# ivanalberico/End-To-End-Self-Supervised-SLAM

Measured on AMD Instinct MI355X. Metric: online refinement steps/sec @640x480, seq_len=60, higher is better.
Workload: dtype f32

## Files before the change

### end-to-end-self-supervised-slam_amd/csrc/conv.hip

```cpp
#include <cassert>
#include <type_traits>

#include "e2e_common.h"

typedef float f4v __attribute__((ext_vector_type(4)));
typedef float f16v __attribute__((ext_vector_type(16)));

#define CBK 16

enum { ACT_NONE = 0, ACT_RELU = 1, ACT_ELU = 2, ACT_DISP = 3 };

struct ConvArgs {
    const float* src0;
    const float* src1;
    const float* w;
    const float* scale;
    const float* shift;
    const float* res;
    float* out;
    int B, Hs, Ws;
    int Cin, C1, up;
    int Hd, Wd;
    int Ncols, ldw;
    int KH, KW, stride, pad, pad_mode;
// ... 1760 lines not shown
#pragma unroll
        for (int i = 0; i < 5; ++i) {
            const int f = tid + TAP_NT * i;
            if (f < 800) *(f4v*)&xs[f * 4] = rx[i];
        }
    };
    if (c_begin < c_end) load_chunk(c_begin);
    const float* ap = dzs + kh_ * 32 + l32;
    const float* bp = xs + (kh_ + wave * 10) * 32 + l32;
    for (int c = c_begin; c < c_end; ++c) {
        __syncthreads();
        store_chunk();
        __syncthreads();
        if (c + 1 < c_end) load_chunk(c + 1);
        constexpr int QB = 4, NQ = 32 / QB;
        float av[2][QB], bv[2][QB][3];
        auto read_q = [&](int set, int qt) {
#pragma unroll
            for (int j = 0; j < QB; ++j) {
                const int ks = QB * qt + j, q0 = (ks >> 2) * 10 + 2 * (ks & 3);
                av[set][j] = ap[2 * ks * 32];
#pragma unroll
                for (int t = 0; t < 3; ++t) bv[set][j][t] = bp[(q0 + t) * 32];
            }
        };
        auto pin_q = [&](int set) {
#pragma unroll
            for (int j = 0; j < QB; ++j) {
                asm volatile("" : "+v"(av[set][j]));
#pragma unroll
                for (int t = 0; t < 3; ++t) asm volatile("" : "+v"(bv[set][j][t]));
            }
        };
        read_q(0, 0);
#pragma unroll
        for (int qt = 0; qt < NQ; ++qt) {
            if (qt + 1 < NQ) read_q((qt + 1) & 1, qt + 1);
            __builtin_amdgcn_sched_barrier(0);
            pin_q(qt & 1);
            __builtin_amdgcn_sched_barrier(0);
#pragma unroll
            for (int j = 0; j < QB; ++j) {
#pragma unroll
                for (int t = 0; t < 3; ++t) acc[t] = __builtin_amdgcn_mfma_f32_32x32x2f32(av[qt & 1][j], bv[qt & 1][j][t], acc[t], 0, 0, 0);
                if (BIAS && want_bias) accb = __builtin_amdgcn_mfma_f32_32x32x2f32(av[qt & 1][j], one, accb, 0, 0, 0);
            }
            __builtin_amdgcn_sched_barrier(0);
        }
    }
    float* slab = a.slabs + (int64_t)blockIdx.z * a.Mpad * a.Npad;
#pragma unroll
    for (int t = 0; t < 3; ++t)
#pragma unroll
        for (int r = 0; r < 16; ++r) {
            const int m = co0 + (r & 3) + 8 * (r >> 2) + 4 * kh_;
            slab[(int64_t)m * a.Npad + (wave * 3 + t) * a.Cin + ci0 + l32] = acc[t][r];
        }
    if (BIAS && want_bias && l32 == 0) {
#pragma unroll
        for (int r = 0; r < 16; ++r) slab[(int64_t)(co0 + (r & 3) + 8 * (r >> 2) + 4 * kh_) * a.Npad + 9 * a.Cin] = accb[r];
    }
}

template <int ZL>
__device__ __forceinline__ void wgrad_reduce_group(const float* __restrict__ slabs, int S, int Mpad, int Npad, int Cout, int Cin, int KH, int KW, int has_bias,
                                                   float* __restrict__ dw, float* __restrict__ dbias, int accumulate, const float* __restrict__ scale,
                                                   int64_t base, int e, int w, f4v (*part)[64]) {
    const int Kconv = KH * KW * Cin, Ng = Kconv + (has_bias ? 1 : 0);
    const int nq = (Ng + 3) / 4;
    const int64_t totalq = (int64_t)Cout * nq;
    const int64_t slab_q = (int64_t)Mpad * Npad / 4;
    const f4v zero = {0.f, 0.f, 0.f, 0.f};
    const int64_t q = base + e;
    const bool on = q < totalq;
    const int m = on ? (int)(q / nq) : 0, n = on ? (int)(q - (int64_t)m * nq) * 4 : 0;
    const f4v* src = (const f4v*)(slabs + (int64_t)m * Npad + n);
    f4v sacc = zero;
    int z = w;
    for (; z + 3 * ZL < S; z += 4 * ZL) {
        f4v v[4];
#pragma unroll
        for (int j = 0; j < 4; ++j) v[j] = on ? src[(int64_t)(z + ZL * j) * slab_q] : zero;
#pragma unroll
        for (int j = 0; j < 4; ++j) sacc += v[j];
    }
    for (; z < S; z += ZL) sacc += on ? src[(int64_t)z * slab_q] : zero;
    part[w][e] = sacc;
    __syncthreads();
    if (w == 0 && on) {
        f4v t = part[0][e];
#pragma unroll
        for (int j = 1; j < ZL; ++j) t += part[j][e];
        const float sc = scale ? scale[m] : 1.f;
#pragma unroll
        for (int k = 0; k < 4; ++k) {
            const int nn = n + k;
            if (nn < Kconv) {
                const int tap = nn / Cin, ci = nn - tap * Cin, kh = tap / KW, kw = tap - kh * KW;
                float* d = dw + (((int64_t)m * Cin + ci) * KH + kh) * KW + kw;
                const float v = scale ? t[k] * sc : t[k];
                *d = accumulate ? *d + v : v;
            } else if (nn == Kconv && dbias) {
                dbias[m] = accumulate ? dbias[m] + t[k] : t[k];
            }
        }
    }
    __syncthreads();
}

template <int ZL>
__global__ __launch_bounds__(64 * ZL) void k_wgrad_reduce(const float* __restrict__ slabs, int S, int Mpad, int Npad, int Cout, int Cin,
                                                         int KH, int KW, int has_bias, float* __restrict__ dw, float* __restrict__ dbias,
                                                         int accumulate, const float* __restrict__ scale) {
    __shared__ f4v part[ZL][64];
    const int64_t totalq = (int64_t)Cout * ((KH * KW * Cin + (has_bias ? 1 : 0) + 3) / 4);
    for (int64_t base = (int64_t)blockIdx.x * 64; base < totalq; base += (int64_t)gridDim.x * 64)
        wgrad_reduce_group<ZL>(slabs, S, Mpad, Npad, Cout, Cin, KH, KW, has_bias, dw, dbias, accumulate, scale, base, threadIdx.x & 63, threadIdx.x >> 6, part);
}

__global__ __launch_bounds__(512) void k_wgrad_reduce_batched(const e2e_wgrad_reduce_desc* __restrict__ d, int n, long long total_items) {
    __shared__ f4v part[8][64];
    const int e = threadIdx.x & 63, w = threadIdx.x >> 6;
    for (long long item = blockIdx.x; item < total_items; item += gridDim.x) {
        int lo = 0, hi = n - 1;
        while (lo < hi) {
            const int mid = (lo + hi + 1) >> 1;
            if (d[mid].first_item <= item) lo = mid; else hi = mid - 1;
        }
        const e2e_wgrad_reduce_desc D = d[lo];
        const long long local = item - D.first_item;
        if (D.zl == 8)
            wgrad_reduce_group<8>(D.slabs, D.S, D.Mpad, D.Npad, D.Cout, D.Cin, D.KH, D.KW, D.has_bias, D.dw, D.dbias, D.accumulate, D.scale, local * 64, e, w, part);
        else
            wgrad_reduce_group<2>(D.slabs, D.S, D.Mpad, D.Npad, D.Cout, D.Cin, D.KH, D.KW, D.has_bias, D.dw, D.dbias, D.accumulate, D.scale,
                                  (local * 4 + (w >> 1)) * 64, e, w & 1, part + 2 * (w >> 1));
    }
}

__global__ __launch_bounds__(256) void k_weight_layouts(const float* __restrict__ w, int Cout, int Cin, int KH, int KW,
                                                        float* __restrict__ wf, int ldf, float* __restrict__ wb, int ldb) {
    const int64_t total = (int64_t)Cout * Cin * KH * KW;
    for (int64_t i = (int64_t)blockIdx.x * 256 + threadIdx.x; i < total; i += (int64_t)gridDim.x * 256) {
        int64_t t = i;
        const int kw = (int)(t % KW); t /= KW;
        const int kh = (int)(t % KH); t /= KH;
        const int ci = (int)(t % Cin); t /= Cin;
        const int co = (int)t;
        const float v = w[i];
        if (wf) wf[((int64_t)(kh * KW + kw) * Cin + ci) * ldf + co] = v;
        if (wb) wb[((int64_t)(kh * KW + kw) * Cout + co) * ldb + ci] = v;
    }
}

__global__ __launch_bounds__(256) void k_weight_layouts_batched(const long long* __restrict__ desc) {
    const long long* d = desc + (int64_t)blockIdx.y * 10;
    const float* __restrict__ w = (const float*)d[0];
    float* __restrict__ wf = (float*)d[1];
    float* __restrict__ wb = (float*)d[2];
    const int Cout = (int)d[3], Cin = (int)d[4], KH = (int)d[5], KW = (int)d[6], ldf = (int)d[7], ldb = (int)d[8];
    const float* __restrict__ bsc = (const float*)d[9];
    const int T = KH * KW;
    constexpr int TMAX = 9, TS = 32;
    __shared__ float tile[TMAX][TS + 1][TS + 1];
    if (T > TMAX) {
        const int64_t total = (int64_t)Cout * Cin * T;
        for (int64_t i = (int64_t)blockIdx.x * 256 + threadIdx.x; i < total; i += (int64_t)gridDim.x * 256) {
            const int tap = (int)(i % T);
            const int64_t r = i / T;
            const int ci = (int)(r % Cin), co = (int)(r / Cin);
            const float v = w[i];
            if (wf) wf[((int64_t)tap * Cin + ci) * ldf + co] = v;
            if (wb) wb[((int64_t)tap * Cout + co) * ldb + ci] = bsc ? v * bsc[co] : v;
        }
        return;
    }
    const int nct = (Cout + TS - 1) / TS, nit = (Cin + TS - 1) / TS;
    for (int t = blockIdx.x; t < nct * nit; t += gridDim.x) {
        const int co0 = (t / nit) * TS, ci0 = (t % nit) * TS;
        const int nci = min(TS, Cin - ci0), nco = min(TS, Cout - co0);
        const int row = nci * T;
        for (int e = threadIdx.x; e < nco * row; e += 256) {
            const int co_l = e / row, rem = e - co_l * row;
            const int ci_l = rem / T, tap = rem - ci_l * T;
            tile[tap][co_l][ci_l] = w[((int64_t)(co0 + co_l) * Cin + ci0) * T + rem];
        }
        __syncthreads();
        if (wf)
            for (int e = threadIdx.x; e < T * nci * nco; e += 256) {
                const int co_l = e % nco, r = e / nco;
                const int ci_l = r % nci, tap = r / nci;
                wf[((int64_t)tap * Cin + ci0 + ci_l) * ldf + co0 + co_l] = tile[tap][co_l][ci_l];
            }
        if (wb)
            for (int e = threadIdx.x; e < T * nco * nci; e += 256) {
                const int ci_l = e % nci, r = e / nci;
                const int co_l = r % nco, tap = r / nco;
                wb[((int64_t)tap * Cout + co0 + co_l) * ldb + ci0 + ci_l] = bsc ? tile[tap][co_l][ci_l] * bsc[co0 + co_l] : tile[tap][co_l][ci_l];
            }
        __syncthreads();
    }
}

__global__ __launch_bounds__(256) void k_act_bwd(const float* __restrict__ dy, const float* __restrict__ y, const float* __restrict__ scale,
                                                 float* __restrict__ dz, int64_t n, int C, int act, int accumulate) {
    for (int64_t i = (int64_t)blockIdx.x * 256 + threadIdx.x; i < n; i += (int64_t)gridDim.x * 256) {
        float g = dy[i];
        const float v = y[i];
        if (act == ACT_RELU) g = v > 0.f ? g : 0.f;
        else if (act == ACT_ELU) g = v > 0.f ? g : g * (v + 1.f);
        else if (act == ACT_DISP) { const float s = (v - 0.01f) * 0.1f; g = g * 10.f * s * (1.f - s); }
        if (scale) g *= scale[i % C];
        dz[i] = accumulate ? dz[i] + g : g;
    }
}

__global__ __launch_bounds__(256) void k_gather_adjoint(const float* __restrict__ dxp, int B, int Hs, int Ws, int Cin, int C1, int up,
                                                        int pp, float* __restrict__ d0, float* __restrict__ d1, int acc0, int acc1,
                                                        const float* __restrict__ x0, int act0, const float* __restrict__ x1, int act1) {
    const int Hp = Hs + 2 * pp, Wp = Ws + 2 * pp, C2 = Cin - C1, Hl = Hs / up, Wl = Ws / up;
    const int64_t n0 = (int64_t)B * Hl * Wl * C1, n1 = (int64_t)B * Hs * Ws * C2;
    for (int64_t i = (int64_t)blockIdx.x * 256 + threadIdx.x; i < n0 + n1; i += (int64_t)gridDim.x * 256) {
        const bool first = i < n0;
        int64_t t = first ? i : i - n0;
        const int Cx = first ? C1 : C2, Hx = first ? Hl : Hs, Wx = first ? Wl : Ws, u = first ? up : 1;
        const int c = (int)(t % Cx); t /= Cx;
        const int x = (int)(t % Wx); t /= Wx;
        const int y = (int)(t % Hx); t /= Hx;
        const int b = (int)t;
        const int cc = first ? c : C1 + c;
        float s = 0.f;
        for (int dy = 0; dy < u; ++dy)
            for (int dx = 0; dx < u; ++dx) {
                const int fy = y * u + dy, fx = x * u + dx;
                int ys[3] = {fy + pp, -1, -1}, xs[3] = {fx + pp, -1, -1};
                if (pp) {
                    if (fy == 1) ys[1] = 0;
                    if (fy == Hs - 2) ys[2] = Hp - 1;
                    if (fx == 1) xs[1] = 0;
                    if (fx == Ws - 2) xs[2] = Wp - 1;
                }
                for (int iy = 0; iy < 3; ++iy)
                    for (int ix = 0; ix < 3; ++ix)
                        if (ys[iy] >= 0 && xs[ix] >= 0) s += dxp[(((int64_t)b * Hp + ys[iy]) * Wp + xs[ix]) * Cin + cc];
            }
        float* d = first ? d0 + i : d1 + (i - n0);
        const int acc = first ? acc0 : acc1;
        if (first ? act0 : act1) s *= act_deriv(first ? x0[i] : x1[i - n0], first ? act0 : act1);
        *d = acc ? *d + s : s;
    }
}

__global__ __launch_bounds__(256) void k_gather_adjoint4(const float* __restrict__ dxp, int B, int Hs, int Ws, int Cin, int C1, int up,
                                                         int pp, float* __restrict__ d0, float* __restrict__ d1, int acc0, int acc1,
                                                         const float* __restrict__ x0, int act0, const float* __restrict__ x1, int act1) {
    const int Hp = Hs + 2 * pp, Wp = Ws + 2 * pp, C2 = Cin - C1, Hl = Hs / up, Wl = Ws / up;
    const unsigned q0 = (unsigned)B * Hl * Wl * (C1 >> 2), q1 = (unsigned)B * Hs * Ws * (C2 >> 2);
    for (unsigned i = blockIdx.x * 256u + threadIdx.x; i < q0 + q1; i += gridDim.x * 256u) {
        const bool first = i < q0;
        unsigned t = first ? i : i - q0;
        const unsigned Cq = (unsigned)(first ? C1 : C2) >> 2, Hx = first ? Hl : Hs, Wx = first ? Wl : Ws;
        const int u = first ? up : 1;
        const unsigned cq = t % Cq; t /= Cq;
        const unsigned x = t % Wx; t /= Wx;
        const unsigned y = t % Hx;
        const unsigned b = t / Hx;
        const int cc = (first ? 0 : C1) + (int)cq * 4;
        f4v s = {0.f, 0.f, 0.f, 0.f};
        for (int dy = 0; dy < u; ++dy)
            for (int dx = 0; dx < u; ++dx) {
                const int fy = (int)y * u + dy, fx = (int)x * u + dx;
                int ys[3] = {fy + pp, -1, -1}, xs[3] = {fx + pp, -1, -1};
                if (pp) {
                    if (fy == 1) ys[1] = 0;
                    if (fy == Hs - 2) ys[2] = Hp - 1;
                    if (fx == 1) xs[1] = 0;
                    if (fx == Ws - 2) xs[2] = Wp - 1;
                }
#pragma unroll
                for (int iy = 0; iy < 3; ++iy)
#pragma unroll
                    for (int ix = 0; ix < 3; ++ix)
                        if (ys[iy] >= 0 && xs[ix] >= 0) s += *(const f4v*)(dxp + (((int64_t)b * Hp + ys[iy]) * Wp + xs[ix]) * Cin + cc);
            }
        const int64_t e = (int64_t)(first ? i : i - q0) * 4;
        const int act = first ? act0 : act1;
        if (act) {
            const f4v xv = *(const f4v*)((first ? x0 : x1) + e);
#pragma unroll
            for (int k = 0; k < 4; ++k) s[k] *= act_deriv(xv[k], act);
        }
        f4v* d = (f4v*)((first ? d0 : d1) + e);
        if (first ? acc0 : acc1) s += *d;
        *d = s;
    }
}

#define HC 16
__global__ __launch_bounds__(256) void k_head_fwd(const float* __restrict__ x, const float* __restrict__ w ,
                                                  const float* __restrict__ bias, float* __restrict__ y, int B, int H, int W, int act) {
    __shared__ float sw[9 * HC];
    for (int i = threadIdx.x; i < 9 * HC; i += 256) {
        const int ci = i / 9, tap = i - ci * 9;
        sw[tap * HC + ci] = w[i];
    }
    __syncthreads();
    const int64_t N = (int64_t)B * H * W;
    const int q = threadIdx.x & 3;
    for (int64_t n0 = (int64_t)blockIdx.x * 64; n0 < N; n0 += (int64_t)gridDim.x * 64) {
        const int64_t n = n0 + (threadIdx.x >> 2);
        const bool on = n < N;
        const int64_t nn = on ? n : N - 1;
        const int b = (int)(nn / ((int64_t)H * W));
        const int r = (int)(nn - (int64_t)b * H * W), h = r / W, ww = r - h * W;
        float acc = 0.f;
#pragma unroll
        for (int kh = 0; kh < 3; ++kh)
#pragma unroll
            for (int kw = 0; kw < 3; ++kw) {
                const int ys = reflect1(h + kh - 1, H), xs = reflect1(ww + kw - 1, W);
                const f4v v = *(const f4v*)(x + (((int64_t)b * H + ys) * W + xs) * HC + q * 4);
                const float* wt = &sw[(kh * 3 + kw) * HC + q * 4];
                acc = fmaf(v[0], wt[0], fmaf(v[1], wt[1], fmaf(v[2], wt[2], fmaf(v[3], wt[3], acc))));
            }
        acc += __shfl_xor(acc, 1, 64);
        acc += __shfl_xor(acc, 2, 64);
        if (on && q == 0) y[n] = apply_act(acc + (bias ? bias[0] : 0.f), act);
    }
}

__global__ __launch_bounds__(256) void k_head_bwd_data(const float* __restrict__ dz, const float* __restrict__ w, float* __restrict__ dx,
                                                       int B, int H, int W, const float* __restrict__ xin, int dact) {
    __shared__ float sw[9 * HC];
    for (int i = threadIdx.x; i < 9 * HC; i += 256) {
        const int ci = i / 9, tap = i - ci * 9;
        sw[tap * HC + ci] = w[i];
    }
    __syncthreads();
    const int64_t N = (int64_t)B * H * W;
    const int cq = threadIdx.x & 3;
    for (int64_t n = (int64_t)blockIdx.x * 64 + (threadIdx.x >> 2); n < N; n += (int64_t)gridDim.x * 64) {
        const int b = (int)(n / ((int64_t)H * W));
        const int r = (int)(n - (int64_t)b * H * W), h = r / W, ww = r - h * W;
        f4v acc = {0.f, 0.f, 0.f, 0.f};
        const int ry = (h == 1) ? 0 : ((h == H - 2) ? H + 1 : -100);
        const int rx = (ww == 1) ? 0 : ((ww == W - 2) ? W + 1 : -100);
        const float* gz = dz + (int64_t)b * H * W;
#pragma unroll
        for (int kh = 0; kh < 3; ++kh)
#pragma unroll
            for (int kw = 0; kw < 3; ++kw) {
                const float* wt = &sw[(kh * 3 + kw) * HC + cq * 4];
                const int qy0 = h - kh + 1, qx0 = ww - kw + 1, qy1 = ry - kh, qx1 = rx - kw;
// ... 112 lines not shown
            const double wgs = (double)tiles * s, per_cu = wgs <= 256 ? 1 : wgs <= 512 ? 2 : wgs <= 768 ? 3 : 0;
            const double f = per_cu == 1 ? 1.0 : per_cu == 2 ? 1.76 : per_cu == 3 ? 2.41 : 2.41 * wgs / 768.0;
            return f * ((double)nchunks / s + 6.0) + (s > 1 ? 4.0 : 0.0);
        };
        if (tiles < 500 && S > 1) {
            int best = S;
            for (int s = S - 2; s <= S + 2; ++s) {
                if (s < 2 || s > 12 || s == S || (nchunks / s) * cb < 288 || tiles * s > 1300) continue;
                if (model(s) < 0.93 * model(best)) best = s;
            }
            S = best;
        }
        c.S = S;
    }
    return c;
}

template <bool TR>
static void launch_tile(ConvArgs& a, int cb, GemmCfg c, dim3 g, hipStream_t st) {
#define X(BM, BN, WM, WN, TM, TN, MAXCB)                                                                                                 \
    if (c.bm == BM && c.bn == BN) {                                                                                                      \
        if constexpr (MAXCB == 32)                                                                                                       \
            if (cb == 32) { hipLaunchKernelGGL((k_conv_gemm<WM, WN, TM, TN, 4, TR, 32>), g, dim3(64 * WM * WN), 0, st, a); return; }     \
        hipLaunchKernelGGL((k_conv_gemm<WM, WN, TM, TN, 4, TR, 16>), g, dim3(64 * WM * WN), 0, st, a);                                   \
        return;                                                                                                                          \
    }
    CONV_TILE_SHAPES(X)
#undef X
    assert(!"launch_tile: shape not in CONV_TILE_SHAPES");
}

template <bool TR>
static void launch_streamk(ConvArgs& a, int cb, int G, float* workspace, hipStream_t st) {
    const int64_t Ntot = (int64_t)a.B * a.Hd * a.Wd;
    SkArgs s;
    s.flags = (unsigned*)workspace;
    s.slabs = workspace + SK_FLAG_FLOATS;
    s.tiles_n = (a.Ncols + 63) / 64;
    s.C = a.KH * a.KW * a.Cin / cb;
    s.I = ((Ntot + 63) / 64) * s.tiles_n * (long long)s.C;
    if (G > SK_MAX_G) G = SK_MAX_G;
    if ((long long)G > s.I) G = (int)s.I;
    s.G = G;
    if (cb == 32) hipLaunchKernelGGL((k_conv_gemm_sk<TR, 32>), dim3(G), dim3(256), 0, st, a, s);
    else hipLaunchKernelGGL((k_conv_gemm_sk<TR, 16>), dim3(G), dim3(256), 0, st, a, s);
}

enum GemmKind { GK_SCALAR, GK_STREAMK, GK_TILE };
enum GemmTail { GT_NONE, GT_SPLITK4, GT_SPLITK, GT_CLS };
struct GemmLaunch { GemmKind kind; GemmTail tail; GemmCfg c; int cb; dim3 g; int G; };

#define CLS_TAP_SLICES 4
static int64_t cls_rows(int B, int Hd, int Wd) { return (int64_t)B * ((Hd + 1) / 2) * ((Wd + 1) / 2); }
static int64_t cls_slab_floats(int B, int Hd, int Wd, int cols) { return CLS_TAP_SLICES * 4 * cls_rows(B, Hd, Wd) * cols; }

template <bool TR>
static GemmLaunch plan_gemm(ConvArgs& a, int vec, float* workspace_all, GemmCfg force) {
    GemmLaunch p{GK_TILE, GT_NONE, GemmCfg{0, 0, 0}, 16, dim3(1), 0};
    const int64_t Ntot = (int64_t)a.B * a.Hd * a.Wd;
    const int K = a.KH * a.KW * a.Cin;
    const int cb = (vec == 4 && a.Cin % 32 == 0 && (a.C1 == a.Cin || a.C1 % 32 == 0)) ? 32 : 16;
    float* workspace = workspace_all ? workspace_all + SK_FLAG_FLOATS : nullptr;
    a.ksplit = 1; a.cps = 0; a.slab = workspace;
    a.bytes0 = (int64_t)a.B * (a.Hs / a.up) * (a.Ws / a.up) * a.C1 * 4;
    a.bytes1 = (int64_t)a.B * a.Hs * a.Ws * (a.Cin - a.C1) * 4;
    a.bytesw = (int64_t)K * a.ldw * 4;
    p.cb = cb;
    if (vec == 1) {
        p.kind = GK_SCALAR;
        p.g = dim3((unsigned)((Ntot + 127) / 128), (unsigned)((a.Ncols + 63) / 64));
        return p;
    }
    if (TR && a.cls) {
        const int64_t Nc = cls_rows(a.B, a.Hd, a.Wd);
        GemmCfg c = choose_cfg(Nc * 4, a.Ncols, (K * 9 / 16 + cb - 1) / cb * cb, cb, false, force.S < 0 ? GemmCfg{0, 0, 0} : force);
        demote_cb16_only(c);
        p.c = c;
        const int64_t total = Ntot * a.Ncols;
        const int64_t cls_wgs = 4 * ((Nc + c.bm - 1) / c.bm) * ((a.Ncols + c.bn - 1) / c.bn);
        if (workspace && cls_wgs < 500 && a.KH == 3 && a.KW == 3 && a.Cin % cb == 0 && a.Ncols % 4 == 0 && total < (1ll << 31) && !a.scale && !a.shift &&
            a.act == ACT_NONE) {
            a.ksplit = CLS_TAP_SLICES; a.cps = a.Cin / cb; a.cls_rows = Nc;
            p.g = dim3((unsigned)(4 * ((Nc + c.bm - 1) / c.bm)), (unsigned)((a.Ncols + c.bn - 1) / c.bn), (unsigned)CLS_TAP_SLICES);
            p.tail = GT_CLS;
            return p;
        }
        p.g = dim3((unsigned)(4 * ((Nc + c.bm - 1) / c.bm)), (unsigned)((a.Ncols + c.bn - 1) / c.bn));
        return p;
    }
    const GemmCfg c = choose_cfg(Ntot, a.Ncols, K, cb, workspace != nullptr, force);
    p.c = c;
    if (c.S < 0 && workspace && vec == 4 && K % cb == 0 && a.Cin % cb == 0) {
        p.kind = GK_STREAMK;
        p.G = -c.S;
        return p;
    }
    if (c.S > 1) {
        const int nchunks = (K + cb - 1) / cb;
        a.cps = (nchunks + c.S - 1) / c.S;
        const int Sz = (nchunks + a.cps - 1) / a.cps;
        a.ksplit = Sz;
        if (Sz > 1) {
            p.g = dim3((unsigned)((Ntot + c.bm - 1) / c.bm), (unsigned)((a.Ncols + c.bn - 1) / c.bn), (unsigned)Sz);
            const int64_t total = Ntot * a.Ncols;
            p.tail = (a.Ncols % 4 == 0 && total < (1ll << 31)) ? GT_SPLITK4 : GT_SPLITK;
            return p;
        }
        a.ksplit = 1; a.cps = 0;
    }
    p.g = dim3((unsigned)((Ntot + c.bm - 1) / c.bm), (unsigned)((a.Ncols + c.bn - 1) / c.bn));
    return p;
}

template <bool TR>
static void launch_gemm_main(ConvArgs& a, const GemmLaunch& p, float* workspace_all, hipStream_t st) {
    if (p.kind == GK_SCALAR) hipLaunchKernelGGL((k_conv_gemm<4, 1, 1, 2, 1, TR, 16>), p.g, dim3(256), 0, st, a);
    else if (p.kind == GK_STREAMK) launch_streamk<TR>(a, p.cb, p.G, workspace_all, st);
    else launch_tile<TR>(a, p.cb, p.c, p.g, st);
}

static void launch_gemm_tail(const ConvArgs& a, const GemmLaunch& p, hipStream_t st) {
    const int64_t total = (int64_t)a.B * a.Hd * a.Wd * a.Ncols;
    if (p.tail == GT_CLS)
        hipLaunchKernelGGL(k_conv_splitk_epilogue_cls, dim3(egrid(total / 4)), dim3(256), 0, st, a.slab, a.cls_rows, a.B, a.Hd, a.Wd, a.Ncols, a.KH, a.KW, a.off,
                           a.res, a.out, a.xin, a.dact, a.pre);
    else if (p.tail == GT_SPLITK4)
        hipLaunchKernelGGL(k_conv_splitk_epilogue4, dim3(egrid(total / 4)), dim3(256), 0, st, a.slab, a.ksplit, (unsigned)(total / 4), a.Ncols, a.scale, a.shift,
                           a.res, a.out, a.act, a.xin, a.dact, a.pre);
    else if (p.tail == GT_SPLITK)
        hipLaunchKernelGGL(k_conv_splitk_epilogue, dim3(egrid(total)), dim3(256), 0, st, a.slab, a.ksplit, total, a.Ncols, a.scale, a.shift, a.res, a.out, a.act,
                           a.xin, a.dact, a.pre);
}

template <bool TR>
static void launch_gemm(ConvArgs a, int vec, float* workspace_all, GemmCfg force, hipStream_t st) {
    const GemmLaunch p = plan_gemm<TR>(a, vec, workspace_all, force);
    launch_gemm_main<TR>(a, p, workspace_all, st);
    launch_gemm_tail(a, p, st);
}

extern "C" {

int e2e_conv_weight_layouts(const float* w, int Cout, int Cin, int KH, int KW, float* w_fwd, int ld_fwd, float* w_bwd,
                            int ld_bwd, void* stream) {
    E2E_REQUIRE(w && Cout > 0 && Cin > 0 && KH > 0 && KW > 0 && (w_fwd || w_bwd), E2E_ERR_ARG, "e2e_conv_weight_layouts: bad argument");
    E2E_REQUIRE((!w_fwd || (ld_fwd >= Cout && ld_fwd % 4 == 0)) && (!w_bwd || (ld_bwd >= Cin && ld_bwd % 4 == 0)), E2E_ERR_ARG,
                "e2e_conv_weight_layouts: leading dimensions must cover the columns and be multiples of 4");
    hipLaunchKernelGGL(k_weight_layouts, dim3(egrid((int64_t)Cout * Cin * KH * KW)), dim3(256), 0, (hipStream_t)stream, w, Cout, Cin, KH,
                       KW, w_fwd, ld_fwd, w_bwd, ld_bwd);
    E2E_LAUNCH_CHECK("e2e_conv_weight_layouts");
    return E2E_OK;
}

int e2e_conv_weight_layouts_batched(const long long* desc, int nlayers, void* stream) {
    E2E_REQUIRE(desc && nlayers > 0 && nlayers <= 65535, E2E_ERR_ARG, "e2e_conv_weight_layouts_batched: bad argument");
    hipLaunchKernelGGL(k_weight_layouts_batched, dim3(256, nlayers), dim3(256), 0, (hipStream_t)stream, desc);
    E2E_LAUNCH_CHECK("e2e_conv_weight_layouts_batched");
    return E2E_OK;
}

int64_t e2e_conv2d_splitk_workspace_floats(int64_t rows, int cols, int K) {
    if (K % 16 != 0) return 0;
    int smax = 1;
    bool sk = false;
    for (int cb = 16; cb <= 32; cb += 16) {
        const GemmCfg c = choose_cfg(rows, cols, K, cb, true);
        if (c.S > smax) smax = c.S;
        if (c.S < 0) sk = true;
    }
    int64_t n = smax > 1 ? (int64_t)smax * rows * cols : 0;
    if (sk && n < (int64_t)SK_MAX_G * 64 * 64) n = (int64_t)SK_MAX_G * 64 * 64;
    return n ? n + SK_FLAG_FLOATS : 0;
}

int64_t e2e_conv2d_bwd_data_workspace_floats(int B, int Hd, int Wd, int cols, int K, int stride) {
    const int64_t plain = e2e_conv2d_splitk_workspace_floats((int64_t)B * Hd * Wd, cols, K);
    if (stride != 2) return plain;
    const int64_t cls = SK_FLAG_FLOATS + cls_slab_floats(B, Hd, Wd, cols);
    return cls > plain ? cls : plain;
}

int64_t e2e_conv_tuned_workspace_floats(int64_t rows, int cols) {
    int64_t n = (int64_t)16 * rows * cols;
    if (n < (int64_t)SK_MAX_G * 64 * 64) n = (int64_t)SK_MAX_G * 64 * 64;
    return n + SK_FLAG_FLOATS;
}
int e2e_conv_workspace_flag_floats(void) { return SK_FLAG_FLOATS; }
int e2e_conv_streamk_error_index(void) { return SK_ERR_INDEX; }

int e2e_conv_gemm_choice(int64_t rows, int cols, int K, int chunk_depth, int allow_split, int* out3) {
    E2E_REQUIRE(out3 && rows > 0 && cols > 0 && K > 0 && (chunk_depth == 16 || chunk_depth == 32), E2E_ERR_ARG, "e2e_conv_gemm_choice: bad argument");
    const GemmCfg c = choose_cfg(rows, cols, K, chunk_depth, allow_split != 0);
    out3[0] = c.bm; out3[1] = c.bn; out3[2] = c.S;
    return E2E_OK;
}

struct ConvGeom { int B, Hs, Ws, Cin, Cout, Ho, Wo, KH, KW, stride, pad, pad_mode, C1, up; float in_sub, in_mul; };
#define GEOM_LAYER(g) ConvGeom g{}; g.B = B; g.Hs = Hs; g.Ws = Ws; g.Cin = Cin; g.Cout = Cout; g.KH = KH; g.KW = KW; g.stride = stride; g.pad = pad; g.pad_mode = pad_mode
#define GEOM_SOURCES(g) g.C1 = C1; g.up = up; g.in_sub = in_sub; g.in_mul = in_mul
#define GEOM_OUTPUT(g) g.Ho = Ho; g.Wo = Wo
#define GEOM_BWD_DATA(g) GEOM_LAYER(g); GEOM_OUTPUT(g)
#define GEOM_BWD_WEIGHT(g) GEOM_LAYER(g); GEOM_OUTPUT(g); GEOM_SOURCES(g)
#define GEOM_WGRAD_QUERY(g) ConvGeom g{}; g.B = B; g.Ho = Ho; g.Wo = Wo; g.Cin = Cin; g.Cout = Cout; g.KH = KH; g.KW = KW
struct FwdOps { const float *src0, *src1, *w_fwd; int ld_fwd; const float *scale, *shift, *residual; float* out; int act; };
struct BwdDataOps { const float* dz; const float* w_bwd; int ld_bwd; float* dxp; int accumulate; const float* x_in; int in_act; const float* pre_add; };
struct WgradIn { const float *dz, *src0, *src1; float* workspace; };

static int conv_fwd_impl(const FwdOps& f, const ConvGeom& g, float* workspace, GemmCfg force, void* stream) {
    const int B = g.B, Hs = g.Hs, Ws = g.Ws, Cin = g.Cin, Cout = g.Cout, KH = g.KH, KW = g.KW, stride = g.stride, pad = g.pad, pad_mode = g.pad_mode;
    const int C1 = g.C1, up = g.up, ld_fwd = f.ld_fwd;
    E2E_REQUIRE(f.src0 && f.w_fwd && f.out && B > 0 && Hs > 0 && Ws > 0 && Cin > 0 && Cout > 0, E2E_ERR_ARG, "e2e_conv2d_fwd: bad argument");
    E2E_REQUIRE(up == 1 || up == 2, E2E_ERR_ARG, "e2e_conv2d_fwd: upsample factor must be 1 or 2");
    E2E_REQUIRE(C1 > 0 && C1 <= Cin && (C1 == Cin || f.src1), E2E_ERR_ARG, "e2e_conv2d_fwd: bad channel split");
    E2E_REQUIRE(pad_mode == 0 || (pad_mode == 1 && pad == 1 && Hs >= 2 && Ws >= 2), E2E_ERR_ARG, "e2e_conv2d_fwd: reflection padding needs pad == 1");
    E2E_REQUIRE(stride == 1 || stride == 2, E2E_ERR_ARG, "e2e_conv2d_fwd: stride must be 1 or 2");
    E2E_REQUIRE(Hs % up == 0 && Ws % up == 0 && ld_fwd % 4 == 0 && ld_fwd >= Cout, E2E_ERR_ARG, "e2e_conv2d_fwd: bad sizes");
    const int vec = (Cin % 16 == 0 && (C1 == Cin || C1 % 16 == 0)) ? 4 : 1;
    E2E_REQUIRE(vec == 4 || (C1 == Cin && up == 1), E2E_ERR_ARG, "e2e_conv2d_fwd: the scalar path (Cin %% 16 != 0) takes a single full-resolution source");
    E2E_REQUIRE((int64_t)B * Hs * Ws * Cin * 4 < (1ll << 30) && (int64_t)KH * KW * Cin * ld_fwd * 4 < (1ll << 31), E2E_ERR_ARG,
                "e2e_conv2d_fwd: activations must stay below 1 GB, weights below 2 GB (32-bit buffer offsets with out-of-range markers)");
    E2E_REQUIRE(vec != 4 || (KH <= 3 && KW <= 3), E2E_ERR_ARG, "e2e_conv2d_fwd: the channel-quad loader takes kernels up to 3 x 3");
    ConvArgs a{};
    a.src0 = f.src0; a.src1 = f.src1; a.w = f.w_fwd; a.scale = f.scale; a.shift = f.shift; a.res = f.residual; a.out = f.out;
    a.B = B; a.Hs = Hs; a.Ws = Ws; a.Cin = Cin; a.C1 = C1; a.up = up;
    a.Hd = (Hs + 2 * pad - KH) / stride + 1; a.Wd = (Ws + 2 * pad - KW) / stride + 1;
    a.Ncols = Cout; a.ldw = ld_fwd; a.KH = KH; a.KW = KW; a.stride = stride; a.pad = pad; a.pad_mode = pad_mode; a.off = 0; a.act = f.act;
    a.in_sub = g.in_sub; a.in_mul = g.in_mul;
    if (!force.bm && KH == 7 && KW == 7 && stride == 2 && pad == 3 && pad_mode == 0 && Cin == 3 && Cout == 64 && C1 == Cin && up == 1 && !f.residual && ld_fwd >= 64) {
        StemArgs t{f.src0, f.w_fwd, f.scale, f.shift, f.out, B, Hs, Ws, a.Hd, a.Wd, ld_fwd, f.act, g.in_sub, g.in_mul};
        hipLaunchKernelGGL(k_conv7x7_stem, dim3((a.Wd + 31) / 32, (a.Hd + 3) / 4, B), dim3(256), 0, (hipStream_t)stream, t);
    }
    else if (!force.bm && KH == 3 && KW == 3 && stride == 1 && pad == 1 && pad_mode == 1 && Cout == 16 && C1 == Cin && !f.scale && !f.residual && ld_fwd >= 16 &&
        ((Cin == 16 && up == 2) || (Cin == 32 && up == 1))) {
        ThinArgs t{f.src0, f.w_fwd, f.shift, f.out, B, Hs / up, Ws / up, Hs, Ws, ld_fwd, f.act, 1, 0};
        if (Cin == 16) hipLaunchKernelGGL((k_conv3x3_thin<16, 2, true, 8>), dim3((Ws + 63) / 64, (Hs + 7) / 8, B), dim3(256), 0, (hipStream_t)stream, t);
        else hipLaunchKernelGGL((k_conv3x3_thin<32, 1, true, 4>), dim3((Ws + 63) / 64, (Hs + 3) / 4, B), dim3(256), 0, (hipStream_t)stream, t);
    } else
        launch_gemm<false>(a, vec, workspace, force, (hipStream_t)stream);
    E2E_LAUNCH_CHECK("e2e_conv2d_fwd");
    return E2E_OK;
}

int e2e_conv2d_fwd(const float* src0, const float* src1, int C1, int up, const float* w_fwd, int ld_fwd, const float* scale,
                   const float* shift, const float* residual, float* out, int B, int Hs, int Ws, int Cin, int Cout, int KH,
                   int KW, int stride, int pad, int pad_mode, int act, float in_sub, float in_mul, float* workspace, void* stream) {
    GEOM_LAYER(g); GEOM_SOURCES(g);
    return conv_fwd_impl(FwdOps{src0, src1, w_fwd, ld_fwd, scale, shift, residual, out, act}, g, workspace, GemmCfg{0, 0, 0}, stream);
}

static bool tuning_ok(int tile_m, int tile_n, int ksplit) {
    if (tile_m == 0) return true;
    if (ksplit < 0) return tile_m == 64 && tile_n == 64 && -ksplit <= SK_MAX_G;
    return tile_max_cb(tile_m, tile_n) != 0 && ksplit >= 1 && ksplit <= 16;
}

int e2e_conv2d_fwd_tuned(const float* src0, const float* src1, int C1, int up, const float* w_fwd, int ld_fwd, const float* scale,
                         const float* shift, const float* residual, float* out, int B, int Hs, int Ws, int Cin, int Cout, int KH,
                         int KW, int stride, int pad, int pad_mode, int act, float in_sub, float in_mul, float* workspace, int tile_m, int tile_n,
                         int ksplit, void* stream) {
    E2E_REQUIRE(tuning_ok(tile_m, tile_n, ksplit), E2E_ERR_ARG, "e2e_conv2d_fwd_tuned: unsupported decomposition %d x %d / %d", tile_m, tile_n, ksplit);
    GEOM_LAYER(g); GEOM_SOURCES(g);
    return conv_fwd_impl(FwdOps{src0, src1, w_fwd, ld_fwd, scale, shift, residual, out, act}, g, workspace, GemmCfg{tile_m, tile_n, ksplit}, stream);
}

static int bwd_data_setup(const BwdDataOps& d, const ConvGeom& g, GemmCfg force, hipStream_t stream, ConvArgs& a, bool& done) {
    const int B = g.B, Hs = g.Hs, Ws = g.Ws, Cin = g.Cin, Cout = g.Cout, Ho = g.Ho, Wo = g.Wo, KH = g.KH, KW = g.KW, stride = g.stride, pad = g.pad;
    const int pad_mode = g.pad_mode, ld_bwd = d.ld_bwd;
    done = false;
    E2E_REQUIRE(d.pre_add == nullptr || pad_mode == 0, E2E_ERR_ARG, "e2e_conv2d_bwd_data: the pre-activation addend takes a zero-padded layer");
    E2E_REQUIRE(d.in_act == 0 || (d.x_in && (d.in_act == ACT_RELU || d.in_act == ACT_ELU) && pad_mode == 0), E2E_ERR_ARG,
                "e2e_conv2d_bwd_data: the fused input-activation derivative takes ReLU / ELU, the activation's output and a zero-padded layer");
    E2E_REQUIRE(d.dz && d.w_bwd && d.dxp && B > 0 && Cin > 0 && Cout > 0 && Cout % 16 == 0, E2E_ERR_ARG, "e2e_conv2d_bwd_data: bad argument (Cout %% 16 == 0)");
    E2E_REQUIRE(ld_bwd % 4 == 0 && ld_bwd >= Cin && (stride == 1 || stride == 2), E2E_ERR_ARG, "e2e_conv2d_bwd_data: bad sizes");
    E2E_REQUIRE((int64_t)B * Ho * Wo * Cout * 4 < (1ll << 30) && (int64_t)KH * KW * Cout * ld_bwd * 4 < (1ll << 31) && KH <= 3 && KW <= 3, E2E_ERR_ARG,
                "e2e_conv2d_bwd_data: gradients must stay below 1 GB, weights below 2 GB (32-bit buffer offsets), kernels up to 3 x 3");
    if (!force.bm && KH == 3 && KW == 3 && stride == 1 && pad == 1 && pad_mode == 1 && Cin == 16 && Cout == 16 && !d.accumulate && !d.in_act && !d.pre_add && ld_bwd >= 16) {
        ThinArgs t{d.dz, d.w_bwd, nullptr, d.dxp, B, Ho, Wo, Hs + 2, Ws + 2, ld_bwd, ACT_NONE, 2, 1};
        hipLaunchKernelGGL((k_conv3x3_thin<16, 1, false, 8>), dim3((Ws + 2 + 63) / 64, (Hs + 2 + 7) / 8, B), dim3(256), 0, stream, t);
        done = true;
        return E2E_OK;
    }
    a = ConvArgs{};
    a.src0 = d.dz; a.src1 = nullptr; a.w = d.w_bwd; a.out = d.dxp;
    a.B = B; a.Hs = Ho; a.Ws = Wo; a.Cin = Cout; a.C1 = Cout; a.up = 1;
    const int pp = pad_mode == 1 ? pad : 0;
    a.Hd = Hs + 2 * pp; a.Wd = Ws + 2 * pp; a.off = pad_mode == 1 ? 0 : pad;
    a.Ncols = Cin; a.ldw = ld_bwd; a.KH = KH; a.KW = KW; a.stride = stride; a.pad = pad; a.pad_mode = 0; a.act = ACT_NONE;
    a.cls = (stride == 2 && cls_rows(B, a.Hd, a.Wd) < (1 << 24)) ? 1 : 0;
    if (a.cls && (KH < 2 || KW < 2) && !d.accumulate)
        (void)hipMemsetAsync(d.dxp, 0, (size_t)B * a.Hd * a.Wd * Cin * sizeof(float), stream);
    if (d.accumulate) a.res = d.dxp;
    a.xin = d.in_act ? d.x_in : nullptr; a.dact = d.in_act; a.pre = d.pre_add;
    return E2E_OK;
}

static int bwd_data_impl(const BwdDataOps& d, const ConvGeom& g, float* workspace, void* stream, GemmCfg force = GemmCfg{0, 0, 0}) {
    ConvArgs a;
    bool done;
    const int rc = bwd_data_setup(d, g, force, (hipStream_t)stream, a, done);
    if (rc != E2E_OK) return rc;
    if (!done) launch_gemm<true>(a, 4, workspace, force, (hipStream_t)stream);
    E2E_LAUNCH_CHECK("e2e_conv2d_bwd_data");
    return E2E_OK;
}

int e2e_conv2d_bwd_data(const float* dz, const float* w_bwd, int ld_bwd, float* dxp, int B, int Hs, int Ws, int Cin, int Cout,
                        int Ho, int Wo, int KH, int KW, int stride, int pad, int pad_mode, float* workspace, void* stream) {
    GEOM_BWD_DATA(g);
    return bwd_data_impl(BwdDataOps{dz, w_bwd, ld_bwd, dxp, 0, nullptr, 0, nullptr}, g, workspace, stream);
// ... 378 lines not shown
```

Baseline: 213.1.

## Rewrite batched weight-layout kernel with flattened tile scheduling and vectorized transposes

Result: faster. 215.2 (median of 6 runs) (+1.0%).

```diff
diff --git a/end-to-end-self-supervised-slam_amd/csrc/conv.hip b/end-to-end-self-supervised-slam_amd/csrc/conv.hip
--- a/end-to-end-self-supervised-slam_amd/csrc/conv.hip
+++ b/end-to-end-self-supervised-slam_amd/csrc/conv.hip
@@ -1936,52 +1936,124 @@
     }
 }
 
-__global__ __launch_bounds__(256) void k_weight_layouts_batched(const long long* __restrict__ desc) {
-    const long long* d = desc + (int64_t)blockIdx.y * 10;
-    const float* __restrict__ w = (const float*)d[0];
-    float* __restrict__ wf = (float*)d[1];
-    float* __restrict__ wb = (float*)d[2];
-    const int Cout = (int)d[3], Cin = (int)d[4], KH = (int)d[5], KW = (int)d[6], ldf = (int)d[7], ldb = (int)d[8];
-    const float* __restrict__ bsc = (const float*)d[9];
-    const int T = KH * KW;
-    constexpr int TMAX = 9, TS = 32;
-    __shared__ float tile[TMAX][TS + 1][TS + 1];
-    if (T > TMAX) {
-        const int64_t total = (int64_t)Cout * Cin * T;
-        for (int64_t i = (int64_t)blockIdx.x * 256 + threadIdx.x; i < total; i += (int64_t)gridDim.x * 256) {
-            const int tap = (int)(i % T);
-            const int64_t r = i / T;
-            const int ci = (int)(r % Cin), co = (int)(r / Cin);
-            const float v = w[i];
-            if (wf) wf[((int64_t)tap * Cin + ci) * ldf + co] = v;
-            if (wb) wb[((int64_t)tap * Cout + co) * ldb + ci] = bsc ? v * bsc[co] : v;
-        }
-        return;
-    }
-    const int nct = (Cout + TS - 1) / TS, nit = (Cin + TS - 1) / TS;
-    for (int t = blockIdx.x; t < nct * nit; t += gridDim.x) {
-        const int co0 = (t / nit) * TS, ci0 = (t % nit) * TS;
-        const int nci = min(TS, Cin - ci0), nco = min(TS, Cout - co0);
-        const int row = nci * T;
-        for (int e = threadIdx.x; e < nco * row; e += 256) {
-            const int co_l = e / row, rem = e - co_l * row;
-            const int ci_l = rem / T, tap = rem - ci_l * T;
-            tile[tap][co_l][ci_l] = w[((int64_t)(co0 + co_l) * Cin + ci0) * T + rem];
-        }
-        __syncthreads();
-        if (wf)
-            for (int e = threadIdx.x; e < T * nci * nco; e += 256) {
-                const int co_l = e % nco, r = e / nco;
-                const int ci_l = r % nci, tap = r / nci;
-                wf[((int64_t)tap * Cin + ci0 + ci_l) * ldf + co0 + co_l] = tile[tap][co_l][ci_l];
-            }
-        if (wb)
-            for (int e = threadIdx.x; e < T * nco * nci; e += 256) {
-                const int ci_l = e % nci, r = e / nci;
-                const int co_l = r % nco, tap = r / nco;
-                wb[((int64_t)tap * Cout + co0 + co_l) * ldb + ci0 + ci_l] = bsc ? tile[tap][co_l][ci_l] * bsc[co0 + co_l] : tile[tap][co_l][ci_l];
-            }
-        __syncthreads();
+constexpr int WL_TS = 32, WL_ELEMS = 1024, WL_MAXL = 256;
+
+template <int T>
+__device__ __forceinline__ void weight_layout_tile(const float* __restrict__ w, float* __restrict__ wf, float* __restrict__ wb, const float* __restrict__ bsc,
+                                                   int Cout, int Cin, int ldf, int ldb, int co0, int ci0, float* tile) {
+    constexpr int R = WL_TS * T + 1;
+    const int nci = min(WL_TS, Cin - ci0), nco = min(WL_TS, Cout - co0);
+    const int lane = threadIdx.x & 63, wave = threadIdx.x >> 6;
+    const int row = nci * T;
+    if ((Cin & 3) == 0 && ((uintptr_t)w & 15) == 0) {
+        const int rot = (lane >> 3) & 3;
+        for (int co_l = wave; co_l < nco; co_l += 4) {
+            const f4v* src = (const f4v*)(w + ((int64_t)(co0 + co_l) * Cin + ci0) * T);
+            float* dst = tile + co_l * R;
+            for (int x = lane; x < row / 4; x += 64) {
+                const f4v v = src[x];
+#pragma unroll
+                for (int s = 0; s < 4; ++s) {
+                    const int k = (s + rot) & 3;
+                    dst[4 * x + k] = k == 0 ? v[0] : k == 1 ? v[1] : k == 2 ? v[2] : v[3];
+                }
+            }
+        }
+    } else {
+        for (int co_l = wave; co_l < nco; co_l += 4) {
+            const float* src = w + ((int64_t)(co0 + co_l) * Cin + ci0) * T;
+            float* dst = tile + co_l * R;
+            for (int x = lane; x < row; x += 64) dst[x] = src[x];
+        }
+    }
+    __syncthreads();
+    const int l32 = threadIdx.x & 31, g = threadIdx.x >> 5;
+    if (wf) {
+        const int co_l = (l32 & 7) * 4, ci_l = g * 4 + (l32 >> 3);
+        if (ci_l < nci && co_l < nco) {
+            const bool quad = co_l + 4 <= nco && (((uintptr_t)wf | (uintptr_t)(ldf * 4)) & 15) == 0;
+            const float* s = tile + co_l * R + ci_l * T;
+#pragma unroll
+            for (int tap = 0; tap < T; ++tap) {
+                const f4v v = {s[tap], s[R + tap], s[2 * R + tap], s[3 * R + tap]};
+                float* o = wf + ((int64_t)tap * Cin + ci0 + ci_l) * ldf + co0 + co_l;
+                if (quad) *(f4v*)o = v;
+                else
+#pragma unroll
+                    for (int k = 0; k < 4; ++k)
+                        if (co_l + k < nco) o[k] = v[k];
+            }
+        }
+    }
+    if (wb) {
+        const int ci_l = (l32 & 7) * 4, co_l = g * 4 + (l32 >> 3);
+        if (co_l < nco && ci_l < nci) {
+            const bool quad = ci_l + 4 <= nci && (((uintptr_t)wb | (uintptr_t)(ldb * 4)) & 15) == 0;
+            const float sc = bsc ? bsc[co0 + co_l] : 1.f;
+            const float* s = tile + co_l * R + ci_l * T;
+#pragma unroll
+            for (int tap = 0; tap < T; ++tap) {
+                f4v v = {s[tap], s[T + tap], s[2 * T + tap], s[3 * T + tap]};
+                if (bsc) v *= sc;
+                float* o = wb + ((int64_t)tap * Cout + co0 + co_l) * ldb + ci0 + ci_l;
+                if (quad) *(f4v*)o = v;
+                else
+#pragma unroll
+                    for (int k = 0; k < 4; ++k)
+                        if (ci_l + k < nci) o[k] = v[k];
+            }
+        }
+    }
+    __syncthreads();
+}
+
+__global__ __launch_bounds__(256) void k_weight_layouts_batched(const long long* __restrict__ desc, int nlayers) {
+    __shared__ float tile[WL_TS * (WL_TS * 9 + 1)];
+    __shared__ int cnt[WL_MAXL], pre[WL_MAXL + 1];
+    for (int i = threadIdx.x; i < nlayers; i += 256) {
+        const long long* d = desc + (int64_t)i * 10;
+        const int Cout = (int)d[3], Cin = (int)d[4], T = (int)d[5] * (int)d[6];
+        cnt[i] = (T == 1 || T == 9) ? ((Cout + WL_TS - 1) / WL_TS) * ((Cin + WL_TS - 1) / WL_TS) : (int)(((int64_t)Cout * Cin * T + WL_ELEMS - 1) / WL_ELEMS);
+    }
+    __syncthreads();
+    for (int i = threadIdx.x; i <= nlayers; i += 256) {
+        int s = 0;
+        for (int j = 0; j < i; ++j) s += cnt[j];
+        pre[i] = s;
+    }
+    __syncthreads();
+    const int total = pre[nlayers];
+    for (int t = blockIdx.x; t < total; t += gridDim.x) {
+        int lo = 0, hi = nlayers - 1;
+        while (lo < hi) {
+            const int mid = (lo + hi + 1) >> 1;
+            if (pre[mid] <= t) lo = mid; else hi = mid - 1;
+        }
+        lo = __builtin_amdgcn_readfirstlane(lo);
+        const int local = t - pre[lo];
+        const long long* d = desc + (int64_t)lo * 10;
+        const float* __restrict__ w = (const float*)d[0];
+        float* __restrict__ wf = (float*)d[1];
+        float* __restrict__ wb = (float*)d[2];
+        const int Cout = (int)d[3], Cin = (int)d[4], KH = (int)d[5], KW = (int)d[6], ldf = (int)d[7], ldb = (int)d[8];
+        const float* __restrict__ bsc = (const float*)d[9];
+        const int T = KH * KW;
+        if (T == 1 || T == 9) {
+            const int nit = (Cin + WL_TS - 1) / WL_TS;
+            const int co0 = (local / nit) * WL_TS, ci0 = (local % nit) * WL_TS;
+            if (T == 9) weight_layout_tile<9>(w, wf, wb, bsc, Cout, Cin, ldf, ldb, co0, ci0, tile);
+            else weight_layout_tile<1>(w, wf, wb, bsc, Cout, Cin, ldf, ldb, co0, ci0, tile);
+        } else {
+            const int64_t total_e = (int64_t)Cout * Cin * T;
+            for (int64_t i = (int64_t)local * WL_ELEMS + threadIdx.x; i < min(total_e, (int64_t)(local + 1) * WL_ELEMS); i += 256) {
+                const int tap = (int)(i % T);
+                const int64_t r = i / T;
+                const int ci = (int)(r % Cin), co = (int)(r / Cin);
+                const float v = w[i];
+                if (wf) wf[((int64_t)tap * Cin + ci) * ldf + co] = v;
+                if (wb) wb[((int64_t)tap * Cout + co) * ldb + ci] = bsc ? v * bsc[co] : v;
+            }
+        }
     }
 }
 
@@ -2400,9 +2472,20 @@
     return E2E_OK;
 }
 
+static int device_cus() {
+    static const int cus = [] {
+        int dev = 0, n = 0;
+        if (hipGetDevice(&dev) != hipSuccess || hipDeviceGetAttribute(&n, hipDeviceAttributeMultiprocessorCount, dev) != hipSuccess || n <= 0) n = 256;
+        return n;
+    }();
+    return cus;
+}
+
 int e2e_conv_weight_layouts_batched(const long long* desc, int nlayers, void* stream) {
-    E2E_REQUIRE(desc && nlayers > 0 && nlayers <= 65535, E2E_ERR_ARG, "e2e_conv_weight_layouts_batched: bad argument");
-    hipLaunchKernelGGL(k_weight_layouts_batched, dim3(256, nlayers), dim3(256), 0, (hipStream_t)stream, desc);
+    E2E_REQUIRE(desc && nlayers > 0, E2E_ERR_ARG, "e2e_conv_weight_layouts_batched: bad argument");
+    const int grid = device_cus() * 8;
+    for (int l0 = 0; l0 < nlayers; l0 += WL_MAXL)
+        hipLaunchKernelGGL(k_weight_layouts_batched, dim3(grid), dim3(256), 0, (hipStream_t)stream, desc + (int64_t)l0 * 10, nlayers - l0 < WL_MAXL ? nlayers - l0 : WL_MAXL);
     E2E_LAUNCH_CHECK("e2e_conv_weight_layouts_batched");
     return E2E_OK;
 }
```
